# pkhungurn/talking-head-anime-4-demo

Hardware: NVIDIA H100
Metric: 512x512 RGBA frames/sec (higher is better)
Workload: dtype f16/tf32 operands (10-bit mantissa), f32 accumulate, f32 storage outside conv operands

## Files before the change

### include/tha4_b200.h

```cpp
#ifndef THA4_B200_H
#define THA4_B200_H

#include <stdint.h>

#ifdef __cplusplus
extern "C" {
#endif

typedef struct tha4_ctx tha4_ctx;

#define THA4_OK 0
#define THA4_ERR_INVALID (-1)
#define THA4_ERR_CUDA (-2)

enum tha4_net {
    THA4_NET_EYEBROW_DECOMPOSER = 0,
    THA4_NET_EYEBROW_MORPHING_COMBINER = 1,
    THA4_NET_FACE_MORPHER = 2,
    THA4_NET_BODY_MORPHER = 3,
    THA4_NET_UPSCALER = 4,
    THA4_NET_SIREN_FACE_MORPHER = 5,
    THA4_NET_SIREN_BODY_MORPHER = 6,
    THA4_NET_COUNT = 7
};
// ... 55 lines not shown
                                       int B, void* stream);
int tha4_siren_morpher_backward(tha4_ctx* ctx, const float* image, const float* pose, int pose_ld, int B,
                                const float* const* grad_outputs, const float* grid_change, const float* alpha,
                                const float* params, float* grads, float* d_image, float* d_pose, void* stream);
int tha4_siren_face_morpher_backward(tha4_ctx* ctx, const float* pose, int pose_ld, int B, const float* grad_output,
                                     const float* params, float* grads, float* d_pose, void* stream);
int tha4_adam_step(tha4_ctx* ctx, float* params, const float* grads, float* exp_avg, float* exp_avg_sq, int64_t n, float lr,
                   float beta1, float beta2, float eps, int step, float grad_scale, void* stream);

int tha4_images_differ(tha4_ctx* ctx, const float* a, const float* b, int64_t n, int* differ, void* stream);

int tha4_frame_to_srgb8(tha4_ctx* ctx, const float* frame, int B, int H, int W, int background, int round_mode, uint8_t* out, void* stream);
int tha4_rgba8_to_poser_image(tha4_ctx* ctx, const uint8_t* rgba, int H, int W, float* out, void* stream);

int tha4_grid_sample(tha4_ctx* ctx, const float* image, const float* grid_change, int N, int C, int H, int W,
                     float* out, int32_t* x0, int32_t* y0, float* tx, float* ty, void* stream);
int tha4_resize_bilinear(tha4_ctx* ctx, const float* in, int N, int C, int Hi, int Wi, int Ho, int Wo, float* out, void* stream);
int tha4_base_grid(int size, float* host_out);
int tha4_test_conv(tha4_ctx* ctx, int kind, const float* x, const float* w, const float* bias, const float* res,
                   int res_mode, int in_up, float* y, int N, int Cin, int H, int W, int Cout, int strict, int ksplit,
                   void* stream);
int tha4_test_conv_norm(tha4_ctx* ctx, int kind, const float* x, int N, int Cin, int H, int W, int norm_C, int groups,
                        const float* gamma, const float* beta, const float* film0, const float* film1, int act,
                        const float* w, const float* bias, const float* res, int res_mode, int Cout, int ksplit,
                        float* y, float* y_from_f16, void* stream);
int tha4_test_conv_norm_ex(tha4_ctx* ctx, int kind, const float* x, int N, int Cin, int H, int W, int norm_C, int groups,
                           const float* gamma, const float* beta, const float* film0, const float* film1, int act,
                           const float* w, const float* bias, const float* res, int res_mode, int Cout, int ksplit,
                           float* y, float* y_from_f16, double* y_stats, int reps, float* us_per_launch, void* stream);
int tha4_test_conv_skip_fold(tha4_ctx* ctx, const float* x, int N, int Cmid, int H, int W, int groups, const float* gamma,
                             const float* beta, const float* film0, const float* film1, int act, const float* w, const float* bias,
                             const float* x2, int Cin2, const float* w_skip, const float* b_skip, int Cout, int ksplit,
                             float* y, double* y_stats, int* folded, int reps, float* us_per_launch, void* stream);
int tha4_test_norm(tha4_ctx* ctx, const float* x, int N, int C, int H, int W, int groups, const float* gamma,
                   const float* beta, const float* film0, const float* film1, int act, int pool, int out_f16, float* y, void* stream);
int tha4_test_tail(tha4_ctx* ctx, int kind, const float* feature, int N, int C, int S, const float* gamma, const float* beta,
                   int groups, int act, const float* head_w, const float* head_b, const int* head_cout, int n_heads,
                   const float* image0, const float* image1, float* const* outputs, int strict, void* stream);
int tha4_test_conv_backward_data(tha4_ctx* ctx, int kind, const float* dy, const float* w, float* dx, int N, int Cin, int H, int W,
                                 int Cout, int strict, void* stream);
int tha4_test_norm_backward(tha4_ctx* ctx, const float* x, int N, int C, int H, int W, const float* gamma, const float* beta,
                            int act, const float* dy, float* dx, void* stream);
int tha4_test_tail_backward(tha4_ctx* ctx, int kind, const float* const* outputs, int N, int S, const float* image0,
                            const float* image1, const float* const* grad_outputs, float* d_head, float* d_image0,
                            float* d_image1, void* stream);
int tha4_test_upscaler_prologue_backward(tha4_ctx* ctx, const float* rest_image, const float* coarse_grid_change, int coarse_size,
                                         int N, const float* d_x0, float* d_rest_image, float* d_coarse_posed_image,
                                         float* d_coarse_grid_change, void* stream);
int tha4_test_group_norm_backward(tha4_ctx* ctx, const float* x, int N, int C, int H, int W, int groups, const float* gamma,
                                  const float* beta, const float* film0, const float* film1, int act, const float* dy, float* dx,
                                  float* d_film, void* stream);
int tha4_test_attention_backward(tha4_ctx* ctx, const float* qkv, const float* dout, int N, int C, int heads, float* dqkv, void* stream);
int tha4_test_group_norm_backward_ex(tha4_ctx* ctx, const void* x, int x_f16, int x_ld, int N, int C, int H, int W, int groups,
                                     const double* stats, int stats_rep, int stats_ld, const float* gamma, const float* beta,
                                     const float* film0, const float* film1, int film1_ld, int film1_off, int act, const float* dy,
                                     int dy_ld, int dy_pool, const float* res, int res_ld, int res_mode, const float* add, int add_ld,
                                     float* dx, int dx_ld, float* d_film, int d_film_ld, void* stream);
int tha4_test_norm_backward_ex(tha4_ctx* ctx, const void* x, int x_f16, int x_ld, int N, int C, int H, int W, const double* stats,
                               int stats_rep, int stats_ld, const float* gamma, const float* beta, int act, const float* dy, int dy_ld,
                               float* dx, int dx_ld, void* stream);
int tha4_test_conv_backward_data_ex(tha4_ctx* ctx, int kind, const float* w, const float* head_b, const int* head_cout, int n_heads,
                                    const float* dy, int dy_ld, const float* add, int add_ld, float* dx, int dx_ld, int N, int Cin,
                                    int H, int W, int Cout, int strict, int workspace, int* split_plan, void* stream);
int tha4_test_linear_backward(tha4_ctx* ctx, const float* dy, int dy_ld, int N, int R, const float* W, int K, const float* pre, int pre_ld,
                              float* dx, int dx_ld, void* stream);
int tha4_test_attention(tha4_ctx* ctx, const float* qkv, int N, int C, int heads, float* out, void* stream);
// ... 26 lines not shown
```

### tha4_b200/_lib.py

```python
import ctypes
import os
import weakref
from typing import Dict, List, Optional, Sequence

import torch
from torch import Tensor

_HERE = os.path.dirname(os.path.abspath(__file__))
LIB_PATH = os.path.join(_HERE, 'libtha4_b200.so')

NET_IDS = {
    'eyebrow_decomposer': 0, 'eyebrow_morphing_combiner': 1, 'face_morpher': 2, 'body_morpher': 3, 'upscaler': 4,
    'siren_face_morpher': 5, 'siren_body_morpher': 6,
}

EXPORTED_SYMBOLS = [
    'tha4_ctx_create', 'tha4_ctx_destroy', 'tha4_last_error', 'tha4_set_option', 'tha4_get_counter', 'tha4_load_net',
    'tha4_eyebrow_decomposer_forward', 'tha4_eyebrow_morphing_combiner_forward', 'tha4_face_morpher_forward',
    'tha4_morpher_forward', 'tha4_upscaler_forward', 'tha4_siren_face_morpher_forward', 'tha4_siren_morpher_forward',
    'tha4_teacher_forward', 'tha4_student_forward', 'tha4_student_forward_io',
    'tha4_bank_create', 'tha4_bank_destroy', 'tha4_bank_set_character', 'tha4_bank_forward', 'tha4_siren_morpher_param_count', 'tha4_siren_morpher_train_step',
    'tha4_siren_face_morpher_param_count', 'tha4_siren_face_morpher_train_step',
    'tha4_siren_morpher_backward', 'tha4_siren_face_morpher_backward',
    'tha4_adam_step', 'tha4_images_differ', 'tha4_frame_to_srgb8', 'tha4_rgba8_to_poser_image', 'tha4_grid_sample', 'tha4_resize_bilinear',
    'tha4_eyebrow_decomposer_backward', 'tha4_eyebrow_morphing_combiner_backward', 'tha4_face_morpher_backward',
    'tha4_morpher_backward', 'tha4_upscaler_backward',
    'tha4_test_conv_backward_data', 'tha4_test_norm_backward', 'tha4_test_tail_backward', 'tha4_test_upscaler_prologue_backward',
    'tha4_test_group_norm_backward', 'tha4_test_attention_backward',
    'tha4_test_group_norm_backward_ex', 'tha4_test_norm_backward_ex', 'tha4_test_conv_backward_data_ex', 'tha4_test_linear_backward',
    'tha4_base_grid', 'tha4_test_conv', 'tha4_test_conv_norm', 'tha4_test_conv_norm_ex', 'tha4_test_conv_skip_fold', 'tha4_test_norm', 'tha4_test_tail', 'tha4_test_attention', 'tha4_test_linear',
    'tha4_test_siren_level', 'tha4_test_sine', 'tha4_test_siren_plan_check',
    'tha4_test_dense_gemm', 'tha4_test_dense_wgrad', 'tha4_test_level_input', 'tha4_test_distill_sine', 'tha4_test_pose_grad',
    'tha4_test_distill_tail',
]

_lib = None


class Tha4Error(RuntimeError):
    pass


def load_library() -> ctypes.CDLL:
    global _lib
    if _lib is not None:
        return _lib
    if not os.path.exists(LIB_PATH):
        raise Tha4Error('tha4_b200: %s is missing -- build it with `python __graft_entry__.py` (nvcc, sm_100a). '
                        'There is no CPU / PyTorch fallback.' % LIB_PATH)
    lib = ctypes.CDLL(LIB_PATH)
    lib.tha4_last_error.restype = ctypes.c_char_p
    lib.tha4_last_error.argtypes = [ctypes.c_void_p]
    lib.tha4_get_counter.restype = ctypes.c_int64
    lib.tha4_get_counter.argtypes = [ctypes.c_void_p, ctypes.c_char_p]
    lib.tha4_set_option.argtypes = [ctypes.c_void_p, ctypes.c_char_p, ctypes.c_int64]
    lib.tha4_siren_morpher_param_count.restype = ctypes.c_int64
    lib.tha4_siren_face_morpher_param_count.restype = ctypes.c_int64
    lib.tha4_adam_step.argtypes = [ctypes.c_void_p, ctypes.c_void_p, ctypes.c_void_p, ctypes.c_void_p, ctypes.c_void_p, ctypes.c_int64,
                                   ctypes.c_float, ctypes.c_float, ctypes.c_float, ctypes.c_float, ctypes.c_int, ctypes.c_float,
                                   ctypes.c_void_p]
    lib.tha4_images_differ.argtypes = [ctypes.c_void_p, ctypes.c_void_p, ctypes.c_void_p, ctypes.c_int64,
                                       ctypes.POINTER(ctypes.c_int), ctypes.c_void_p]
    P, I, I64 = ctypes.c_void_p, ctypes.c_int, ctypes.c_int64
# ... 461 lines not shown
```

### tha4_b200/csrc/capi.cu

```cuda
#include "../../include/tha4_b200.h"
#include "nets.cuh"
#include "siren.cuh"
#include "profiler.cuh"
#include "distill.cuh"
#include <atomic>
#include <cstring>
#include <map>
#include <tuple>
#include <vector>

namespace tha4 {
std::atomic<long> g_kernel_launches{0};
bool g_use_pdl = true;
thread_local AllocSink* g_alloc_sink = nullptr;
void* tracked_malloc(size_t bytes) {
    void* p = nullptr;
    THA4_CUDA_CHECK(cudaMalloc(&p, std::max<size_t>(bytes, 16)));
    if (g_alloc_sink) g_alloc_sink->ptrs.push_back(p);
    return p;
}
}

using namespace tha4;

// ... 198 lines not shown

int tha4_ctx_destroy(tha4_ctx* ctx) {
    if (!ctx) return THA4_ERR_INVALID;
    cudaSetDevice(ctx->device);
    cudaDeviceSynchronize();
    if (ctx->flag) cudaFree(ctx->flag);
    if (ctx->loss_acc) cudaFree(ctx->loss_acc);
    if (ctx->pose_stage) cudaFree(ctx->pose_stage);
    if (ctx->capture_stream) cudaStreamDestroy(ctx->capture_stream);
    if (ctx->side) { cudaStreamDestroy(ctx->side); cudaEventDestroy(ctx->ev_fork); cudaEventDestroy(ctx->ev_join); }
    if (ctx->stats_base) cudaFree(ctx->stats_base);
    ctx->drop_graphs();
    delete ctx;
    return THA4_OK;
}

const char* tha4_last_error(const tha4_ctx* ctx) { return ctx ? ctx->err.c_str() : g_create_err.c_str(); }

int tha4_set_option(tha4_ctx* ctx, const char* name, int64_t value) {
    return guarded(ctx, [&] {
        cudaDeviceSynchronize();
        ctx->drop_graphs();
        if (!strcmp(name, "strict")) { ctx->strict = value ? 1 : 0; }
        else if (!strcmp(name, "cuda_graphs")) ctx->use_graphs = value ? 1 : 0;
        else if (!strcmp(name, "side_stream")) ctx->side_streams = value ? 1 : 0;
        else if (!strcmp(name, "tcgen05")) conv_enable_tc(value != 0);
        else if (!strcmp(name, "cluster_splitk")) conv_tc_enable_cluster(value != 0);
        else if (!strcmp(name, "halo_conv")) conv_halo_enable(value != 0);
        else if (!strcmp(name, "tma_store")) conv_halo_enable_tma_store(value != 0);
        else if (!strcmp(name, "halo_m256")) { THA4_REQUIRE(value >= -1 && value <= 1, "halo_m256: -1, 0 or 1"); conv_halo_set_m256((int)value); }
        else if (!strcmp(name, "halo_ctas")) { THA4_REQUIRE(value == -1 || value == 1 || value == 2, "halo_ctas: -1, 1 or 2"); conv_halo_set_ctas((int)value); }
        else if (!strcmp(name, "halo_cs")) { THA4_REQUIRE(value == -1 || value == 1 || value == 2, "halo_cs: -1, 1 or 2"); conv_halo_set_cs((int)value); }
        else if (!strcmp(name, "skip_fold")) unet_set_skip_fold(value != 0);
        else if (!strcmp(name, "siren_tc")) siren_tc_enable(value != 0);
        else if (!strcmp(name, "tc_stride2")) conv_tc_enable_stride2(value != 0);
        else if (!strcmp(name, "small_bn")) conv_tc_enable_small_bn(value != 0);
        else if (!strcmp(name, "attn_split16")) attention_enable_split16(value != 0);
        else if (!strcmp(name, "tail_persist")) tail_tc_enable_persist(value != 0);
        else if (!strcmp(name, "attn_mma")) attention_enable_mma(value != 0);
        else if (!strcmp(name, "half_operands")) ctx->half_operands = value ? 1 : 0;
        else if (!strcmp(name, "pdl")) g_use_pdl = value != 0;
        else if (!strcmp(name, "profile")) { prof_enable(value != 0); if (value == 2) prof_reset(); }
        else if (!strcmp(name, "microbatch")) { THA4_REQUIRE(value >= 1 && value <= 1024, "microbatch range"); ctx->microbatch = (int)value; }
        else throw std::runtime_error(std::string("tha4: unknown option ") + name);
    });
}

int64_t tha4_get_counter(const tha4_ctx* ctx, const char* name) {
    if (!strcmp(name, "kernel_launches")) return g_kernel_launches.load();
    {
        static const char* cats[] = {"conv", "norm", "tail", "attn", "glue", "siren"};
        static const char* whats[] = {"us", "launches", "flops", "bytes"};
        if (!strncmp(name, "prof_", 5))
            for (int w = 0; w < 4; ++w)
                for (int c = 0; c < 6; ++c)
                    if (std::string(name) == std::string("prof_") + whats[w] + "_" + cats[c]) {
                        try { return (int64_t)prof_read(c, w); } catch (...) { return -1; }
                    }
    }
    if (ctx && !strcmp(name, "graph_replays")) return (int64_t)ctx->graph_replays;
    if (ctx && !strcmp(name, "graph_captures")) return (int64_t)ctx->graph_captures;
    if (ctx && !strcmp(name, "graph_failures")) return (int64_t)ctx->graph_failures;
    if (ctx && !strcmp(name, "workspace_bytes")) return (int64_t)(ctx->persist.bytes() + ctx->scratch.bytes());
    return -1;
}

// ... 687 lines not shown
        const bool fold = unet_skip_fold() && conv_halo_supported(fw, fa);
        View sk = mk(N, H, W, Cout);
        ConvArgs sa; sa.in = x16; sa.out = sk;
        a.res = sk; a.res_mode = RES_SAME;
        const size_t wsf = std::max(conv_workspace_floats(sw, sa), conv_workspace_floats(cw, a));
        float* ws = wsf ? ctx->scratch.alloc(wsf) : nullptr;
        for (ConvArgs* c : {&sa, &a}) { c->ws = ws; c->ws_floats = wsf; }
        auto run = [&] {
            if (fold) { conv_forward(fw, fa, s); return; }
            if (y_stats) THA4_CUDA_CHECK(cudaMemsetAsync(yo.stats, 0, (size_t)N * Cout * 2 * sizeof(double), s));
            conv_forward(sw, sa, s);
            conv_forward(cw, a, s);
        };
        run();
        if (y_stats) THA4_CUDA_CHECK(cudaMemcpyAsync(y_stats, yo.stats, (size_t)N * Cout * 2 * sizeof(double), cudaMemcpyDeviceToDevice, s));
        if (folded) *folded = fold ? 1 : 0;
        if (reps > 0) {
            cudaEvent_t e0, e1;
            THA4_CUDA_CHECK(cudaEventCreate(&e0)); THA4_CUDA_CHECK(cudaEventCreate(&e1));
            THA4_CUDA_CHECK(cudaEventRecord(e0, s));
            for (int i = 0; i < reps; ++i) run();
            THA4_CUDA_CHECK(cudaEventRecord(e1, s));
            THA4_CUDA_CHECK(cudaEventSynchronize(e1));
            float ms = 0.0f;
            THA4_CUDA_CHECK(cudaEventElapsedTime(&ms, e0, e1));
            cudaEventDestroy(e0); cudaEventDestroy(e1);
            if (us_per_launch) *us_per_launch = 1000.0f * ms / reps;
        }
        nhwc_to_nchw(yo, y, s);
        THA4_CUDA_CHECK(cudaStreamSynchronize(s));
    });
}

int tha4_test_norm(tha4_ctx* ctx, const float* x, int N, int C, int H, int W, int groups, const float* gamma,
                   const float* beta, const float* film0, const float* film1, int act, int pool, int out_f16, float* y, void* stream) {
    return guarded(ctx, [&] {
        cudaStream_t s = (cudaStream_t)stream;
        begin_pass(ctx, s);
        Runtime rt = make_rt(ctx, stream);
        Pool* P = &ctx->persist;
        View xin; xin.N = N; xin.H = H; xin.W = W; xin.C = C; xin.ld = C; xin.p = P->alloc((size_t)N * H * W * C);
        xin.stats_rep = 2; xin.stats_rep_stride = (long)N * C * 2;
        xin.stats = rt.alloc_stats((size_t)2 * N * C * 2); xin.stats_ld = C;
        nchw_to_nhwc(make_img(x, N, C, H, W), xin, s);
        norm_stats(xin, s);
        View yo = xin; yo.stats = nullptr;
        if (pool) { yo.H = H / 2; yo.W = W / 2; }
        yo.p = P->alloc((size_t)N * yo.H * yo.W * C);
        if (out_f16) {
            View y16 = yo; y16.f16 = 1; y16.p = P->alloc(((size_t)N * yo.H * yo.W * C + 1) / 2);
            norm_apply_fused(xin, groups, gamma, beta, film0, film1, 2 * C, act == ACT_SILU ? ACT_SILU_FAST : act, pool, nullptr, y16, s, 1);
            convert_f32(y16, yo, s);
        } else {
            norm_apply_fused(xin, groups, gamma, beta, film0, film1, 2 * C, act, pool, nullptr, yo, s, 0);
        }
        nhwc_to_nchw(yo, y, s);
    });
}

int tha4_test_tail(tha4_ctx* ctx, int kind, const float* feature, int N, int C, int S, const float* gamma, const float* beta,
                   int groups, int act, const float* head_w, const float* head_b, const int* head_cout, int n_heads,
                   const float* image0, const float* image1, float* const* outputs, int strict, void* stream) {
    return guarded(ctx, [&] {
        cudaStream_t s = (cudaStream_t)stream;
        begin_pass(ctx, s);
        Runtime rt = make_rt(ctx, stream);
// ... 405 lines not shown
```

### tha4_b200/csrc/conv.cuh

```cuda
#pragma once
#include "common.cuh"

namespace tha4 {

constexpr int CONV_MAX_TAPS = 16;
constexpr int CONV_MAX_PHASES = 4;

enum ResMode { RES_NONE = 0, RES_SAME = 1, RES_UP2 = 2, RES_DOWN2 = 3 };

struct ConvWeights {
    float* w = nullptr;
    mutable __half* w16 = nullptr;
    mutable float w16_scale = 1.0f;
    float* bias = nullptr;
    int cin = 0, cout = 0, cin_pad = 0, cout_pad = 0;
    int ntaps = 0, nphase = 1;
    bool dynamic = false;
    bool tf32_rounded = false;
    int stride = 1;
    int out_mul = 1;
    signed char dy[CONV_MAX_PHASES][CONV_MAX_TAPS];
    signed char dx[CONV_MAX_PHASES][CONV_MAX_TAPS];
    signed char ph_oy[CONV_MAX_PHASES], ph_ox[CONV_MAX_PHASES];
    int cin2 = 0, cin2_pad = 0;
// ... 30 lines not shown
    View res;
    int res_mode = RES_NONE;
    int strict = 0;
    int ksplit = 0;
    float* ws = nullptr;
    size_t ws_floats = 0;
};

size_t conv_workspace_floats(const ConvWeights& cw, const ConvArgs& a);

void conv_forward(const ConvWeights& cw, const ConvArgs& a, cudaStream_t s);
void conv_mma_forward(const ConvWeights& cw, const ConvArgs& a, cudaStream_t s);
bool conv_tc_supported(const ConvWeights& cw, const ConvArgs& a);
void conv_tc_forward(const ConvWeights& cw, const ConvArgs& a, cudaStream_t s);
bool conv_fuses_stats(const ConvWeights& cw, const ConvArgs& a);
bool conv_tc_fuses_stats(const ConvWeights& cw, const ConvArgs& a);
int conv_tc_split_plan(const ConvWeights& cw, const ConvArgs& a);
bool conv_halo_supported(const ConvWeights& cw, const ConvArgs& a);
void conv_halo_forward(const ConvWeights& cw, const ConvArgs& a, cudaStream_t s);
void conv_halo_enable(bool on);
void conv_halo_enable_tma_store(bool on);
void conv_halo_set_ctas(int mode);
void conv_halo_set_cs(int mode);
void conv_halo_set_m256(int mode);
void conv_halo_debug_dump();
void conv_enable_tc(bool on);
bool conv_tc_enabled();
void conv_make_half(const ConvWeights& cw, cudaStream_t s);
void conv_make_fold(ConvWeights& fold, const ConvWeights& conv3, const ConvWeights& conv1x1, cudaStream_t s);
void conv_tc_enable_cluster(bool on);
void conv_tc_enable_small_bn(bool on);
void conv_tc_enable_stride2(bool on);

}
```

### tha4_b200/csrc/nets.cu

```cuda
#include "nets.cuh"
#include <algorithm>
#include <cmath>
#include <cstdlib>

namespace tha4 {

Pool::~Pool() { for (void* p : all_) cudaFree(p); }

float* Pool::alloc(size_t nfloats) {
    size_t bytes = ((nfloats * sizeof(float) + 255) / 256) * 256;
    if (bytes == 0) bytes = 256;
    Bucket& bk = buckets_[bytes];
    if (bk.next < bk.blocks.size()) return reinterpret_cast<float*>(bk.blocks[bk.next++]);
    void* p = nullptr;
    THA4_CUDA_CHECK(cudaMalloc(&p, bytes));
    bk.blocks.push_back(p);
    bk.next = bk.blocks.size();
    all_.push_back(p);
    total_ += bytes;
    return reinterpret_cast<float*>(p);
}

void Pool::reset() { for (auto& kv : buckets_) kv.second.next = 0; }

// ... 670 lines not shown
                rt.stream = rt.side;
                try { run_conv_tc(rt, w.skip, x.h, nullptr, sk); } catch (...) { rt.stream = main_stream; throw; }
                rt.stream = main_stream;
                THA4_CUDA_CHECK(cudaEventRecord(rt.ev_join, rt.side));
            } else {
                run_conv_tc(rt, w.skip, x.h, nullptr, sk);
            }
        }
        View xpool;
        if (mode == 2) {
            View t0 = make_view16(rt.scratch, B, x.f.H / 2, x.f.W / 2, w.cin);
            xpool = make_view(rt.scratch, B, x.f.H / 2, x.f.W / 2, w.cin);
            run_norm(rt, x.f, w.norm0, 32, nullptr, nullptr, 0, act, 1, nullptr, t0, nullptr, &xpool);
            run_conv_tc(rt, w.conv0, t0, nullptr, h0);
        } else {
            const ConvNormIn n0 = norm_in(x.f, w.norm0, 32, act);
            run_conv_tc(rt, w.conv0, x.h, &n0, h0);
        }
        const ConvNormIn n1 = norm_in(h0.f, w.norm1, 32, act, w.film0, film1 + w.film1_off, film1_total);
        if (fold) {
            run_conv_tc(rt, w.fold, h0.h, &n1, out, nullptr, RES_NONE, &x.h);
        } else if (w.has_skip) {
            THA4_REQUIRE(mode == 0, "res_block: skip conv only on same-resolution blocks");
            if (rt.side) THA4_CUDA_CHECK(cudaStreamWaitEvent(rt.stream, rt.ev_join, 0));
            run_conv_tc(rt, w.conv1, h0.h, &n1, out, &sk.f, RES_SAME);
        } else {
            if (mode == 2) run_conv_tc(rt, w.conv1, h0.h, &n1, out, &xpool, RES_SAME);
            else run_conv_tc(rt, w.conv1, h0.h, &n1, out, &x.f, mode == 0 ? RES_SAME : RES_UP2);
        }
    }

    void attn_block(const AttnW& w, const Tens& x, const Tens& out) {
        rt.scratch->reset();
        Tens qkv = make_act(tape ? rt.persist : rt.scratch, rt, x.f.N, x.f.H, x.f.W, 3 * x.f.C, true, false, false);
        const ConvNormIn n = norm_in(x.f, w.norm, 32, ACT_NONE);
        run_conv_tc(rt, w.qkv, x.h, &n, qkv);
        if (tape) tape->attn[&w] = {op_view(x), qkv.f};
        View a = make_view(rt.scratch, x.f.N, x.f.H, x.f.W, x.f.C);
        attention_forward(qkv.f, 8, a, rt.stream, true);
        run_conv_tc(rt, w.proj, a, nullptr, out, &x.f, RES_SAME);
    }
};

}

void UNetNet::forward_fused(Runtime& rt, const ImgView& image, const float* coarse_posed, const float* coarse_grid, int coarse_size,
                            const float* pose, int pose_ld, float* const* outputs, UNetTape* tape) {
    const int B = image.N;
    cudaStream_t s = rt.stream;
    Pool* P = rt.persist;
    rt.scratch->reset();

    float* c1 = P->alloc((size_t)B * 256);
    float* c2 = P->alloc((size_t)B * 256);
    float* film1 = P->alloc((size_t)B * film1_total_);
    cudaStream_t ls = s;
    if (rt.side) {
        THA4_CUDA_CHECK(cudaEventRecord(rt.ev_fork, s));
        THA4_CUDA_CHECK(cudaStreamWaitEvent(rt.side, rt.ev_fork, 0));
        ls = rt.side;
    }
    linear_forward(pose, pose_ld, B, 6, cond_w0_, cond_b0_, 256, 0, c1, 256, ls);
    linear_forward(c1, 256, B, 256, cond_w2_, cond_b2_, 256, 1, c2, 256, ls);
    linear_forward(c2, 256, B, 256, film1_w_, film1_b_, film1_total_, 1, film1, film1_total_, ls);
    if (rt.side) THA4_CUDA_CHECK(cudaEventRecord(rt.ev_join, rt.side));
    if (tape) { tape->c1 = c1; tape->c2 = c2; tape->film1 = film1; }
    UNetFused F{rt, film1, film1_total_, tape};

// ... 99 lines not shown
```

Before: 178.7.

## Fuse attention block into one clustered kernel with DSMEM K/V exchange

Replaces the three-launch attention block (norm plus qkv 1x1 conv, attention, proj conv plus residual) with a single kernel. It runs a 16-CTA cluster per image, one CTA per head and half of the tokens, and uses distributed shared memory to exchange K/V halves and per-head outputs before the projection. It also writes output stats and the f16 copy in the epilogue. The goal is to avoid the round trips of qkv and attention output through global memory and to save launch overhead, at the cost of a fixed 16x16x256 shape and a large cluster that may not place well.

Result: faster. 183.7 (median of 6 runs) (+2.8%).

```diff
diff --git a/include/tha4_b200.h b/include/tha4_b200.h
--- a/include/tha4_b200.h
+++ b/include/tha4_b200.h
@@ -111,6 +111,10 @@
                              const float* beta, const float* film0, const float* film1, int act, const float* w, const float* bias,
                              const float* x2, int Cin2, const float* w_skip, const float* b_skip, int Cout, int ksplit,
                              float* y, double* y_stats, int* folded, int reps, float* us_per_launch, void* stream);
+int tha4_test_attn_block(tha4_ctx* ctx, const float* x, int N, int in_reps, const float* gamma, const float* beta,
+                         const float* w_qkv, const float* b_qkv, const float* w_proj, const float* b_proj, int out_mode, int out_ld,
+                         int out_reps, float* y, float* y16, double* y_stats, float* qkv, int* fused, int reps, float* us_per_launch,
+                         void* stream);
 int tha4_test_norm(tha4_ctx* ctx, const float* x, int N, int C, int H, int W, int groups, const float* gamma,
                    const float* beta, const float* film0, const float* film1, int act, int pool, int out_f16, float* y, void* stream);
 int tha4_test_tail(tha4_ctx* ctx, int kind, const float* feature, int N, int C, int S, const float* gamma, const float* beta,
diff --git a/tha4_b200/_lib.py b/tha4_b200/_lib.py
--- a/tha4_b200/_lib.py
+++ b/tha4_b200/_lib.py
@@ -28,7 +28,7 @@
     'tha4_test_conv_backward_data', 'tha4_test_norm_backward', 'tha4_test_tail_backward', 'tha4_test_upscaler_prologue_backward',
     'tha4_test_group_norm_backward', 'tha4_test_attention_backward',
     'tha4_test_group_norm_backward_ex', 'tha4_test_norm_backward_ex', 'tha4_test_conv_backward_data_ex', 'tha4_test_linear_backward',
-    'tha4_base_grid', 'tha4_test_conv', 'tha4_test_conv_norm', 'tha4_test_conv_norm_ex', 'tha4_test_conv_skip_fold', 'tha4_test_norm', 'tha4_test_tail', 'tha4_test_attention', 'tha4_test_linear',
+    'tha4_base_grid', 'tha4_test_conv', 'tha4_test_conv_norm', 'tha4_test_conv_norm_ex', 'tha4_test_conv_skip_fold', 'tha4_test_attn_block', 'tha4_test_norm', 'tha4_test_tail', 'tha4_test_attention', 'tha4_test_linear',
     'tha4_test_siren_level', 'tha4_test_sine', 'tha4_test_siren_plan_check',
     'tha4_test_dense_gemm', 'tha4_test_dense_wgrad', 'tha4_test_level_input', 'tha4_test_distill_sine', 'tha4_test_pose_grad',
     'tha4_test_distill_tail',
diff --git a/tha4_b200/csrc/attention_block.cu b/tha4_b200/csrc/attention_block.cu
--- /dev/null
+++ b/tha4_b200/csrc/attention_block.cu
@@ -0,0 +1,363 @@
+#include "conv.cuh"
+#include "ops.cuh"
+#include "profiler.cuh"
+#include "conv_tc_device.cuh"
+
+namespace tha4 {
+namespace {
+
+constexpr int AB_L = 256, AB_C = 256, AB_D = 32, AB_HEADS = 8;
+constexpr int AB_CS = 2 * AB_HEADS;
+constexpr int AB_T = AB_L / 2;
+constexpr int AB_THREADS = 256;
+constexpr int XP = AB_C + 8;
+constexpr int KH_P = AB_D + 8, VT_P = AB_L + 8;
+constexpr int SM_X = 0;
+constexpr int SM_Q = SM_X + AB_T * XP * 2;
+constexpr int SM_K = SM_Q + AB_T * KH_P * 2;
+constexpr int SM_VT = SM_K + AB_L * KH_P * 2;
+constexpr int SM_WQ = SM_VT + AB_D * VT_P * 2;
+constexpr int SM_WP = SM_WQ + 3 * AB_D * XP * 2;
+constexpr int SM_HA = SM_WP + AB_D * XP * 2;
+constexpr int SM_CHS = SM_HA + 2 * AB_C * 2;
+constexpr int SM_RED = SM_CHS + AB_C * 16;
+constexpr int SM_BYTES = SM_RED + 8 * AB_D * 8;
+static_assert(SM_BYTES <= 227 * 1024, "shared memory budget");
+static_assert(3 * AB_D * XP >= AB_T * KH_P, "O_h staging fits in the qkv weight rows");
+
+struct AbParams {
+    tcdev::TcParams xf;
+    const __half* x; int x_ld;
+    const __half* wq; int wq_ld; const float* bq; float sq;
+    const __half* wp; int wp_ld; const float* bp; float sp;
+    const float* res; int res_ld;
+    float* out; int out_ld;
+    __half* out16; int out16_ld;
+    double* stats; int stats_ld, stats_rep; long stats_rep_stride;
+    float* qkv; int qkv_ld;
+    int pre_w;
+};
+
+__device__ __forceinline__ uint32_t pack_h2(float a, float b) {
+    const __half2 h = __floats2half2_rn(a, b);
+    return *reinterpret_cast<const uint32_t*>(&h);
+}
+__device__ __forceinline__ void mma_16816(float (&c)[4], const uint32_t (&a)[4], uint32_t b0, uint32_t b1) {
+    asm volatile("mma.sync.aligned.m16n8k16.row.col.f32.f16.f16.f32 {%0, %1, %2, %3}, {%4, %5, %6, %7}, {%8, %9}, {%0, %1, %2, %3};\n"
+                 : "+f"(c[0]), "+f"(c[1]), "+f"(c[2]), "+f"(c[3]) : "r"(a[0]), "r"(a[1]), "r"(a[2]), "r"(a[3]), "r"(b0), "r"(b1));
+}
+__device__ __forceinline__ void cp_async16(uint32_t dst, const void* src) {
+    asm volatile("cp.async.cg.shared.global [%0], [%1], 16;\n" :: "r"(dst), "l"(src) : "memory");
+}
+__device__ __forceinline__ void cluster_sync() {
+    asm volatile("barrier.cluster.arrive.release.aligned;\n" ::: "memory");
+    asm volatile("barrier.cluster.wait.acquire.aligned;\n" ::: "memory");
+}
+__device__ __forceinline__ uint32_t peer_addr(uint32_t local, int rank) {
+    uint32_t r;
+    asm volatile("mapa.shared::cluster.u32 %0, %1, %2;\n" : "=r"(r) : "r"(local), "r"(rank));
+    return r;
+}
+__device__ __forceinline__ float tf32_trunc(float v) { return __uint_as_float(__float_as_uint(v) & 0xffffe000u); }
+
+__global__ void __launch_bounds__(AB_THREADS, 1) attn_block_kernel(const __grid_constant__ AbParams p) {
+    extern __shared__ __align__(16) uint8_t sm[];
+    const int tid = threadIdx.x, warp = tid >> 5, lane = tid & 31, g = lane >> 2, t = lane & 3;
+    const int rank = blockIdx.z % AB_CS, n = blockIdx.z / AB_CS;
+    const int h = rank % AB_HEADS, half = rank / AB_HEADS, partner = rank ^ AB_HEADS;
+    const int t0 = half * AB_T;
+    const uint32_t s_base = tc::smem_u32(sm);
+    asm volatile("barrier.cluster.arrive.relaxed.aligned;\n" ::: "memory");
+
+    auto load_w = [&] {
+        for (int j = tid; j < 4 * AB_D * (AB_C / 8); j += AB_THREADS) {
+            const int r = j >> 5, c8 = (j & 31) * 8;
+            if (r < 3 * AB_D) {
+                const __half* src = p.wq + (long)((r >> 5) * AB_C + h * AB_D + (r & 31)) * p.wq_ld + c8;
+                cp_async16(s_base + SM_WQ + (r * XP + c8) * 2, src);
+            } else {
+                const int rp = r - 3 * AB_D;
+                cp_async16(s_base + SM_WP + (rp * XP + c8) * 2, p.wp + (long)(h * AB_D + rp) * p.wp_ld + c8);
+            }
+        }
+        asm volatile("cp.async.commit_group;\n" ::: "memory");
+    };
+    if (p.pre_w) load_w();
+    pdl_trigger();
+    pdl_wait();
+    if (!p.pre_w) load_w();
+
+    {
+        const __half* xs = p.x + ((long)n * AB_L + t0) * p.x_ld;
+        for (int j = tid; j < AB_T * (AB_C / 8); j += AB_THREADS) {
+            const int r = j >> 5, c8 = (j & 31) * 8;
+            cp_async16(s_base + SM_X + (r * XP + c8) * 2, xs + (long)r * p.x_ld + c8);
+        }
+        asm volatile("cp.async.commit_group;\n" ::: "memory");
+    }
+    __half* hA = reinterpret_cast<__half*>(sm + SM_HA);
+    __half* hB = hA + AB_C;
+    tcdev::xf_build_coef<AB_THREADS, 1>(p.xf, n, tid, hA, hB, reinterpret_cast<double2*>(sm + SM_CHS), 0, AB_C);
+    asm volatile("cp.async.wait_all;\n" ::: "memory");
+    __syncthreads();
+    {
+        uint8_t* row = sm + SM_X + (tid >> 1) * XP * 2;
+        const int j0 = (tid & 1) * 16;
+        tcdev::xf_chunks<8>(row, 0, j0, 0, p.xf, hA, hB, false);
+        tcdev::xf_chunks<8>(row, 0, j0 + 8, 0, p.xf, hA, hB, false);
+    }
+    __syncthreads();
+
+    const uint32_t* xw = reinterpret_cast<const uint32_t*>(sm + SM_X);
+    const int m0 = 16 * warp;
+    {
+        float acc[12][4];
+#pragma unroll
+        for (int nj = 0; nj < 12; ++nj) acc[nj][0] = acc[nj][1] = acc[nj][2] = acc[nj][3] = 0.0f;
+        const uint32_t* ww = reinterpret_cast<const uint32_t*>(sm + SM_WQ);
+#pragma unroll 2
+        for (int ks = 0; ks < AB_C / 16; ++ks) {
+            uint32_t a[4];
+            const int lo = (m0 + g) * (XP / 2) + 8 * ks + t, hi = lo + 8 * (XP / 2);
+            a[0] = xw[lo]; a[1] = xw[hi]; a[2] = xw[lo + 4]; a[3] = xw[hi + 4];
+#pragma unroll
+            for (int nj = 0; nj < 12; ++nj) {
+                const int br = (8 * nj + g) * (XP / 2) + 8 * ks + t;
+                mma_16816(acc[nj], a, ww[br], ww[br + 4]);
+            }
+        }
+        const float scale = 1.0f / sqrtf(sqrtf((float)AB_D));
+        uint32_t* qw = reinterpret_cast<uint32_t*>(sm + SM_Q);
+        asm volatile("barrier.cluster.wait.aligned;\n" ::: "memory");
+#pragma unroll
+        for (int nj = 0; nj < 12; ++nj) {
+            const int part = nj >> 2, d = 8 * (nj & 3) + 2 * t;
+            const int gch = part * AB_C + h * AB_D + d;
+            const float b0 = __ldg(p.bq + gch), b1 = __ldg(p.bq + gch + 1);
+#pragma unroll
+            for (int e = 0; e < 2; ++e) {
+                const int rl = m0 + g + 8 * e, r = t0 + rl;
+                const float v0 = acc[nj][2 * e] * p.sq + b0, v1 = acc[nj][2 * e + 1] * p.sq + b1;
+                if (p.qkv) *reinterpret_cast<float2*>(p.qkv + ((long)n * AB_L + r) * p.qkv_ld + gch) = make_float2(v0, v1);
+                if (part == 0) {
+                    qw[(rl * KH_P + d) >> 1] = pack_h2(v0 * scale, v1 * scale);
+                } else if (part == 1) {
+                    const uint32_t kv = pack_h2(v0 * scale, v1 * scale);
+                    const uint32_t a = s_base + SM_K + (r * KH_P + d) * 2;
+                    asm volatile("st.shared.b32 [%0], %1;\n" :: "r"(a), "r"(kv) : "memory");
+                    asm volatile("st.shared::cluster.b32 [%0], %1;\n" :: "r"(peer_addr(a, partner)), "r"(kv) : "memory");
+                } else {
+                    const __half2 vh = __floats2half2_rn(v0, v1);
+                    const unsigned short u0 = __half_as_ushort(__low2half(vh)), u1 = __half_as_ushort(__high2half(vh));
+                    const uint32_t a0 = s_base + SM_VT + (d * VT_P + r) * 2, a1 = a0 + VT_P * 2;
+                    asm volatile("st.shared.b16 [%0], %1;\n" :: "r"(a0), "h"(u0) : "memory");
+                    asm volatile("st.shared.b16 [%0], %1;\n" :: "r"(a1), "h"(u1) : "memory");
+                    asm volatile("st.shared::cluster.b16 [%0], %1;\n" :: "r"(peer_addr(a0, partner)), "h"(u0) : "memory");
+                    asm volatile("st.shared::cluster.b16 [%0], %1;\n" :: "r"(peer_addr(a1, partner)), "h"(u1) : "memory");
+                }
+            }
+        }
+    }
+    cluster_sync();
+
+    {
+        const uint32_t* qw = reinterpret_cast<const uint32_t*>(sm + SM_Q);
+        const uint32_t* kw = reinterpret_cast<const uint32_t*>(sm + SM_K);
+        const uint32_t* vw = reinterpret_cast<const uint32_t*>(sm + SM_VT);
+        uint32_t* os = reinterpret_cast<uint32_t*>(sm + SM_WQ);
+        const int q0 = m0;
+        uint32_t qa[2][4];
+#pragma unroll
+        for (int ks = 0; ks < 2; ++ks) {
+            const int lo = ((q0 + g) * KH_P) / 2 + 8 * ks + t, hi = ((q0 + g + 8) * KH_P) / 2 + 8 * ks + t;
+            qa[ks][0] = qw[lo]; qa[ks][1] = qw[hi]; qa[ks][2] = qw[lo + 4]; qa[ks][3] = qw[hi + 4];
+        }
+        float sc[AB_L / 8][4];
+#pragma unroll
+        for (int j = 0; j < AB_L / 8; ++j) {
+            sc[j][0] = sc[j][1] = sc[j][2] = sc[j][3] = 0.0f;
+            const int krow = ((8 * j + g) * KH_P) >> 1;
+#pragma unroll
+            for (int ks = 0; ks < 2; ++ks)
+                mma_16816(sc[j], qa[ks], kw[krow + 8 * ks + t], kw[krow + 8 * ks + t + 4]);
+        }
+        float mx0 = -INFINITY, mx1 = -INFINITY;
+#pragma unroll
+        for (int j = 0; j < AB_L / 8; ++j) { mx0 = fmaxf(mx0, fmaxf(sc[j][0], sc[j][1])); mx1 = fmaxf(mx1, fmaxf(sc[j][2], sc[j][3])); }
+        mx0 = fmaxf(mx0, __shfl_xor_sync(0xffffffffu, mx0, 1)); mx0 = fmaxf(mx0, __shfl_xor_sync(0xffffffffu, mx0, 2));
+        mx1 = fmaxf(mx1, __shfl_xor_sync(0xffffffffu, mx1, 1)); mx1 = fmaxf(mx1, __shfl_xor_sync(0xffffffffu, mx1, 2));
+        float l0 = 0.0f, l1 = 0.0f;
+        constexpr float LOG2E = 1.4426950408889634f;
+        const float mb0 = mx0 * LOG2E, mb1 = mx1 * LOG2E;
+#pragma unroll
+        for (int j = 0; j < AB_L / 8; ++j) {
+            sc[j][0] = exp2f(fmaf(sc[j][0], LOG2E, -mb0)); sc[j][1] = exp2f(fmaf(sc[j][1], LOG2E, -mb0));
+            sc[j][2] = exp2f(fmaf(sc[j][2], LOG2E, -mb1)); sc[j][3] = exp2f(fmaf(sc[j][3], LOG2E, -mb1));
+            l0 += sc[j][0] + sc[j][1]; l1 += sc[j][2] + sc[j][3];
+        }
+        l0 += __shfl_xor_sync(0xffffffffu, l0, 1); l0 += __shfl_xor_sync(0xffffffffu, l0, 2);
+        l1 += __shfl_xor_sync(0xffffffffu, l1, 1); l1 += __shfl_xor_sync(0xffffffffu, l1, 2);
+        float oc[AB_D / 8][4];
+#pragma unroll
+        for (int nd = 0; nd < AB_D / 8; ++nd) oc[nd][0] = oc[nd][1] = oc[nd][2] = oc[nd][3] = 0.0f;
+#pragma unroll
+        for (int kk = 0; kk < AB_L / 16; ++kk) {
+            uint32_t pa[4];
+            pa[0] = pack_h2(sc[2 * kk][0], sc[2 * kk][1]); pa[1] = pack_h2(sc[2 * kk][2], sc[2 * kk][3]);
+            pa[2] = pack_h2(sc[2 * kk + 1][0], sc[2 * kk + 1][1]); pa[3] = pack_h2(sc[2 * kk + 1][2], sc[2 * kk + 1][3]);
+#pragma unroll
+            for (int nd = 0; nd < AB_D / 8; ++nd) {
+                const int vrow = ((8 * nd + g) * VT_P + 16 * kk) >> 1;
+                mma_16816(oc[nd], pa, vw[vrow + t], vw[vrow + t + 4]);
+            }
+        }
+        const float i0 = 1.0f / l0, i1 = 1.0f / l1;
+#pragma unroll
+        for (int nd = 0; nd < AB_D / 8; ++nd) {
+            os[((q0 + g) * KH_P + 8 * nd + 2 * t) >> 1] = pack_h2(tf32_trunc(oc[nd][0] * i0), tf32_trunc(oc[nd][1] * i0));
+            os[((q0 + g + 8) * KH_P + 8 * nd + 2 * t) >> 1] = pack_h2(tf32_trunc(oc[nd][2] * i1), tf32_trunc(oc[nd][3] * i1));
+        }
+    }
+    __syncthreads();
+
+    for (int j = tid; j < AB_T * (AB_D / 8); j += AB_THREADS) {
+        const int r = j >> 2, c4 = j & 3;
+        const uint4 v = *reinterpret_cast<const uint4*>(sm + SM_WQ + (r * KH_P + 8 * c4) * 2);
+        const uint32_t local = s_base + SM_X + (r * XP + h * AB_D + 8 * c4) * 2;
+#pragma unroll
+        for (int rk = 0; rk < AB_HEADS; ++rk)
+            asm volatile("st.shared::cluster.v4.b32 [%0], {%1, %2, %3, %4};\n"
+                         :: "r"(peer_addr(local, rk + AB_HEADS * half)), "r"(v.x), "r"(v.y), "r"(v.z), "r"(v.w) : "memory");
+    }
+    cluster_sync();
+
+    float acc[4][4];
+#pragma unroll
+    for (int nj = 0; nj < 4; ++nj) acc[nj][0] = acc[nj][1] = acc[nj][2] = acc[nj][3] = 0.0f;
+    {
+        const uint32_t* ww = reinterpret_cast<const uint32_t*>(sm + SM_WP);
+#pragma unroll 4
+        for (int ks = 0; ks < AB_C / 16; ++ks) {
+            uint32_t a[4];
+            const int lo = (m0 + g) * (XP / 2) + 8 * ks + t, hi = lo + 8 * (XP / 2);
+            a[0] = xw[lo]; a[1] = xw[hi]; a[2] = xw[lo + 4]; a[3] = xw[hi + 4];
+#pragma unroll
+            for (int nj = 0; nj < 4; ++nj) {
+                const int br = (8 * nj + g) * (XP / 2) + 8 * ks + t;
+                mma_16816(acc[nj], a, ww[br], ww[br + 4]);
+            }
+        }
+    }
+    float su[4][2], sq[4][2];
+#pragma unroll
+    for (int nj = 0; nj < 4; ++nj) {
+        const int ch = h * AB_D + 8 * nj + 2 * t;
+        const float b0 = __ldg(p.bp + ch), b1 = __ldg(p.bp + ch + 1);
+        su[nj][0] = su[nj][1] = sq[nj][0] = sq[nj][1] = 0.0f;
+#pragma unroll
+        for (int e = 0; e < 2; ++e) {
+            const long pix = (long)n * AB_L + t0 + m0 + g + 8 * e;
+            const float2 rr = *reinterpret_cast<const float2*>(p.res + pix * p.res_ld + ch);
+            float v0 = acc[nj][2 * e] * p.sp, v1 = acc[nj][2 * e + 1] * p.sp;
+            v0 += b0; v1 += b1;
+            v0 += rr.x; v1 += rr.y;
+            if (p.out) *reinterpret_cast<float2*>(p.out + pix * p.out_ld + ch) = make_float2(v0, v1);
+            if (p.out16) *reinterpret_cast<__half2*>(p.out16 + pix * p.out16_ld + ch) = __floats2half2_rn(v0, v1);
+            su[nj][0] += v0; su[nj][1] += v1; sq[nj][0] += v0 * v0; sq[nj][1] += v1 * v1;
+        }
+    }
+    if (p.stats) {
+        float2* red = reinterpret_cast<float2*>(sm + SM_RED);
+#pragma unroll
+        for (int nj = 0; nj < 4; ++nj)
+#pragma unroll
+            for (int c = 0; c < 2; ++c) {
+                float a = su[nj][c], b = sq[nj][c];
+#pragma unroll
+                for (int off = 4; off < 32; off <<= 1) { a += __shfl_xor_sync(0xffffffffu, a, off); b += __shfl_xor_sync(0xffffffffu, b, off); }
+                if (g == 0) red[warp * AB_D + 8 * nj + 2 * t + c] = make_float2(a, b);
+            }
+        __syncthreads();
+        if (tid < AB_D) {
+            double a = 0.0, b = 0.0;
+#pragma unroll
+            for (int w = 0; w < AB_THREADS / 32; ++w) { const float2 v = red[w * AB_D + tid]; a += (double)v.x; b += (double)v.y; }
+            double* d = p.stats + (long)(blockIdx.z % p.stats_rep) * p.stats_rep_stride + ((long)n * p.stats_ld + h * AB_D + tid) * 2;
+            atomicAdd(d, a); atomicAdd(d + 1, b);
+        }
+    }
+}
+
+bool g_attn_fuse = true;
+
+int max_clusters() {
+    static int n[THA4_MAX_DEVICES];
+    static bool known[THA4_MAX_DEVICES];
+    const int d = current_device();
+    if (!known[d]) {
+        THA4_CUDA_CHECK(cudaFuncSetAttribute(attn_block_kernel, cudaFuncAttributeMaxDynamicSharedMemorySize, SM_BYTES));
+        THA4_CUDA_CHECK(cudaFuncSetAttribute(attn_block_kernel, cudaFuncAttributeNonPortableClusterSizeAllowed, 1));
+        cudaLaunchConfig_t cfg{};
+        cfg.gridDim = dim3(1, 1, AB_CS); cfg.blockDim = dim3(AB_THREADS); cfg.dynamicSmemBytes = SM_BYTES;
+        cudaLaunchAttribute attr;
+        attr.id = cudaLaunchAttributeClusterDimension;
+        attr.val.clusterDim.x = 1; attr.val.clusterDim.y = 1; attr.val.clusterDim.z = AB_CS;
+        cfg.attrs = &attr; cfg.numAttrs = 1;
+        int c = 0;
+        if (cudaOccupancyMaxActiveClusters(&c, attn_block_kernel, &cfg) != cudaSuccess) { (void)cudaGetLastError(); c = 0; }
+        n[d] = c; known[d] = true;
+    }
+    return n[d];
+}
+
+}
+
+void attn_block_enable_fuse(bool on) { g_attn_fuse = on; }
+
+bool attn_block_fused_for(int N) { return g_attn_fuse && N <= max_clusters(); }
+
+void attn_block_forward(const ConvWeights& qkv, const ConvWeights& proj, const View& x16, const ConvNormIn& nin, const View& res,
+                        const View& out, const View& out16, const View* qkv_out, cudaStream_t s) {
+    THA4_REQUIRE(x16.f16 && x16.H * x16.W == AB_L && x16.C == AB_C, "attn_block: the input is an f16 view of 256 tokens x 256 channels");
+    THA4_REQUIRE(qkv.ntaps == 1 && qkv.nphase == 1 && qkv.cin == AB_C && qkv.cout == 3 * AB_C && proj.ntaps == 1 && proj.nphase == 1 &&
+                 proj.cin == AB_C && proj.cout == AB_C && AB_C / AB_HEADS == AB_D, "attn_block: 1x1 convs 256 -> 768 and 256 -> 256, 8 heads of 32");
+    THA4_REQUIRE(qkv.w16 && proj.w16 && qkv.bias && proj.bias, "attn_block: the f16 weight copies and the biases");
+    THA4_REQUIRE(qkv.cin_pad % 8 == 0 && proj.cin_pad % 8 == 0 && (((uintptr_t)qkv.w16) & 15) == 0 && (((uintptr_t)proj.w16) & 15) == 0,
+                 "attn_block: weight alignment");
+    THA4_REQUIRE(x16.ld % 8 == 0 && (((uintptr_t)x16.p) & 15) == 0, "attn_block: input alignment (16-byte rows)");
+    THA4_REQUIRE(nin.on && nin.C == AB_C && nin.groups > 0 && AB_C % nin.groups == 0 && nin.stats && nin.gamma && nin.beta &&
+                 !nin.film0 && !nin.film1, "attn_block: a pending GroupNorm of the input");
+    THA4_REQUIRE(res.p && !res.f16 && res.N == x16.N && res.H * res.W == AB_L && res.C == AB_C && res.ld % 2 == 0 && (((uintptr_t)res.p) & 7) == 0,
+                 "attn_block: fp32 residual geometry / alignment");
+    THA4_REQUIRE(out.p || out16.p, "attn_block: no output");
+    THA4_REQUIRE(out.N == x16.N && out.H * out.W == AB_L && out.C == AB_C, "attn_block: output geometry");
+    if (out.p) THA4_REQUIRE(!out.f16 && out.ld % 2 == 0 && (((uintptr_t)out.p) & 7) == 0, "attn_block: fp32 output alignment");
+    if (out16.p)
+        THA4_REQUIRE(out16.f16 && out16.N == out.N && out16.H * out16.W == AB_L && out16.C == AB_C && out16.ld % 2 == 0 &&
+                     (((uintptr_t)out16.p) & 3) == 0, "attn_block: f16 output geometry / alignment");
+    if (qkv_out) THA4_REQUIRE(!qkv_out->f16 && qkv_out->N == x16.N && qkv_out->H * qkv_out->W == AB_L && qkv_out->C == 3 * AB_C &&
+                              qkv_out->ld % 2 == 0 && (((uintptr_t)qkv_out->p) & 7) == 0, "attn_block: qkv output geometry / alignment");
+    AbParams p{};
+    p.xf.in_stats = nin.stats; p.xf.in_stats_ld = nin.stats_ld; p.xf.in_stats_rep = std::max(1, nin.stats_rep);
+    p.xf.in_stats_rep_stride = nin.stats_rep_stride;
+    p.xf.xf_C = AB_C; p.xf.xf_groups = nin.groups; p.xf.xf_act = nin.act;
+    THA4_REQUIRE(nin.act == ACT_NONE, "attn_block: GroupNorm without activation");
+    p.xf.xf_inv_cnt = 1.0 / ((double)AB_L * (AB_C / nin.groups));
+    p.xf.xf_gamma = nin.gamma; p.xf.xf_beta = nin.beta;
+    p.x = x16.hp(); p.x_ld = x16.ld;
+    p.wq = qkv.w16; p.wq_ld = qkv.cin_pad; p.bq = qkv.bias; p.sq = 1.0f / qkv.w16_scale;
+    p.wp = proj.w16; p.wp_ld = proj.cin_pad; p.bp = proj.bias; p.sp = 1.0f / proj.w16_scale;
+    p.res = res.p; p.res_ld = res.ld;
+    p.out = out.p; p.out_ld = out.ld;
+    p.out16 = out16.p ? out16.hp() : nullptr; p.out16_ld = out16.ld;
+    p.stats = out.stats; p.stats_ld = out.stats_ld; p.stats_rep = std::max(1, out.stats_rep); p.stats_rep_stride = out.stats_rep_stride;
+    p.qkv = qkv_out ? qkv_out->p : nullptr; p.qkv_ld = qkv_out ? qkv_out->ld : 0;
+    p.pre_w = (qkv.dynamic || proj.dynamic) ? 0 : 1;
+    ProfScope prof(PROF_ATTN, s);
+    prof_add_work(PROF_ATTN, (double)x16.N * (2.0 * AB_L * AB_C * 4 * AB_C + 4.0 * AB_L * AB_L * AB_C), 0.0);
+    THA4_REQUIRE(max_clusters() > 0, "attn_block: the device cannot place a 16-CTA cluster of this kernel");
+    launch_pdl(attn_block_kernel, dim3(1, 1, AB_CS * x16.N), dim3(AB_THREADS), SM_BYTES, s, AB_CS, p);
+    THA4_LAUNCH_CHECK();
+}
+
+}
diff --git a/tha4_b200/csrc/capi.cu b/tha4_b200/csrc/capi.cu
--- a/tha4_b200/csrc/capi.cu
+++ b/tha4_b200/csrc/capi.cu
@@ -254,6 +254,7 @@
         else if (!strcmp(name, "halo_ctas")) { THA4_REQUIRE(value == -1 || value == 1 || value == 2, "halo_ctas: -1, 1 or 2"); conv_halo_set_ctas((int)value); }
         else if (!strcmp(name, "halo_cs")) { THA4_REQUIRE(value == -1 || value == 1 || value == 2, "halo_cs: -1, 1 or 2"); conv_halo_set_cs((int)value); }
         else if (!strcmp(name, "skip_fold")) unet_set_skip_fold(value != 0);
+        else if (!strcmp(name, "attn_fuse")) attn_block_enable_fuse(value != 0);
         else if (!strcmp(name, "siren_tc")) siren_tc_enable(value != 0);
         else if (!strcmp(name, "tc_stride2")) conv_tc_enable_stride2(value != 0);
         else if (!strcmp(name, "small_bn")) conv_tc_enable_small_bn(value != 0);
@@ -1007,6 +1008,92 @@
     });
 }
 
+int tha4_test_attn_block(tha4_ctx* ctx, const float* x, int N, int in_reps, const float* gamma, const float* beta,
+                         const float* w_qkv, const float* b_qkv, const float* w_proj, const float* b_proj, int out_mode, int out_ld,
+                         int out_reps, float* y, float* y16, double* y_stats, float* qkv, int* fused, int reps, float* us_per_launch,
+                         void* stream) {
+    return guarded(ctx, [&] {
+        cudaStream_t s = (cudaStream_t)stream;
+        begin_pass(ctx, s);
+        Runtime rt = make_rt(ctx, stream);
+        Pool* P = &ctx->persist;
+        constexpr int C = 256, HW = 16;
+        THA4_REQUIRE(N >= 1 && in_reps >= 1 && out_reps >= 1 && out_ld >= C && out_ld % 8 == 0 && (out_mode & 3) != 0,
+                     "test_attn_block: arguments");
+        AllocSink sink;
+        ConvWeights wq, wp;
+        {
+            SinkScope own(&sink);
+            conv_set_pack_rounding(true);
+            for (int k = 0; k < 2; ++k) {
+                ConvWeights& c = k ? wp : wq;
+                conv_describe(c, CONV_1x1, C, k ? C : 3 * C);
+                c.tf32_rounded = true;
+                c.w = reinterpret_cast<float*>(tracked_malloc(conv_packed_floats(c) * sizeof(float)));
+                THA4_CUDA_CHECK(cudaMemsetAsync(c.w, 0, conv_packed_floats(c) * sizeof(float), s));
+                conv_pack(c, CONV_1x1, k ? w_proj : w_qkv, C, 0, s);
+                conv_make_half(c, s);
+            }
+        }
+        wq.bias = const_cast<float*>(b_qkv); wp.bias = const_cast<float*>(b_proj);
+        View xin; xin.N = N; xin.H = HW; xin.W = HW; xin.C = C; xin.ld = C; xin.p = P->alloc((size_t)N * HW * HW * C);
+        xin.stats_rep = in_reps; xin.stats_rep_stride = (long)N * C * 2; xin.stats_ld = C;
+        xin.stats = rt.alloc_stats((size_t)in_reps * N * C * 2);
+        THA4_CUDA_CHECK(cudaMemsetAsync(xin.stats, 0, (size_t)in_reps * N * C * 2 * sizeof(double), s));
+        THA4_CUDA_CHECK(cudaMemcpyAsync(xin.p, x, (size_t)N * HW * HW * C * sizeof(float), cudaMemcpyDeviceToDevice, s));
+        norm_stats(xin, s);
+        View x16 = xin; x16.f16 = 1; x16.stats = nullptr; x16.p = P->alloc((size_t)N * HW * HW * C / 2);
+        convert_f16(xin, x16, s);
+        const size_t on = (size_t)N * HW * HW * out_ld;
+        View of; of.N = N; of.H = HW; of.W = HW; of.C = out_ld; of.ld = out_ld; of.p = P->alloc(on);
+        View oh = of; oh.f16 = 1; oh.p = P->alloc(on / 2);
+        THA4_CUDA_CHECK(cudaMemsetAsync(of.p, 0xff, on * sizeof(float), s));
+        THA4_CUDA_CHECK(cudaMemsetAsync(oh.p, 0xff, on * sizeof(__half), s));
+        const size_t stn = (size_t)out_reps * N * out_ld * 2;
+        of.stats = rt.alloc_stats(stn); of.stats_ld = out_ld; of.stats_rep = out_reps; of.stats_rep_stride = (long)N * out_ld * 2;
+        View o32 = of.slice(out_ld - C, C), o16 = oh.slice(out_ld - C, C);
+        if (!(out_mode & 1)) o32.p = nullptr;
+        if (!(out_mode & 2)) o16.p = nullptr;
+        ConvNormIn nin;
+        nin.on = true; nin.C = C; nin.groups = 32; nin.act = ACT_NONE; nin.gamma = gamma; nin.beta = beta;
+        nin.stats = xin.stats; nin.stats_ld = C; nin.stats_rep = in_reps; nin.stats_rep_stride = xin.stats_rep_stride;
+        View qv; qv.N = N; qv.H = HW; qv.W = HW; qv.C = 3 * C; qv.ld = 3 * C; qv.p = P->alloc((size_t)N * HW * HW * 3 * C);
+        View av = xin; av.stats = nullptr; av.p = P->alloc((size_t)N * HW * HW * C);
+        const bool fuse = attn_block_fused_for(N);
+        ConvArgs a; a.in = x16; a.out = qv; a.nin = nin;
+        ConvArgs b; b.in = av; b.out = o32; b.out16 = o16; b.res = xin; b.res_mode = RES_SAME;
+        const size_t wsf = std::max(conv_workspace_floats(wq, a), conv_workspace_floats(wp, b));
+        float* ws = wsf ? ctx->scratch.alloc(wsf) : nullptr;
+        for (ConvArgs* c : {&a, &b}) { c->ws = ws; c->ws_floats = wsf; }
+        auto run = [&] {
+            THA4_CUDA_CHECK(cudaMemsetAsync(of.stats, 0, stn * sizeof(double), s));
+            if (fuse) { attn_block_forward(wq, wp, x16, nin, xin, o32, o16, qkv ? &qv : nullptr, s); return; }
+            conv_forward(wq, a, s);
+            attention_forward(qv, 8, av, s, true);
+            conv_forward(wp, b, s);
+        };
+        run();
+        if (fused) *fused = fuse ? 1 : 0;
+        if (reps > 0) {
+            cudaEvent_t e0, e1;
+            THA4_CUDA_CHECK(cudaEventCreate(&e0)); THA4_CUDA_CHECK(cudaEventCreate(&e1));
+            THA4_CUDA_CHECK(cudaEventRecord(e0, s));
+            for (int i = 0; i < reps; ++i) run();
+            THA4_CUDA_CHECK(cudaEventRecord(e1, s));
+            THA4_CUDA_CHECK(cudaEventSynchronize(e1));
+            float ms = 0.0f;
+            THA4_CUDA_CHECK(cudaEventElapsedTime(&ms, e0, e1));
+            cudaEventDestroy(e0); cudaEventDestroy(e1);
+            if (us_per_launch) *us_per_launch = 1000.0f * ms / reps;
+        }
+        if (y) THA4_CUDA_CHECK(cudaMemcpyAsync(y, of.p, on * sizeof(float), cudaMemcpyDeviceToDevice, s));
+        if (y16) { View t = of; t.stats = nullptr; t.p = y16; convert_f32(oh, t, s); }
+        if (y_stats) THA4_CUDA_CHECK(cudaMemcpyAsync(y_stats, of.stats, stn * sizeof(double), cudaMemcpyDeviceToDevice, s));
+        if (qkv) THA4_CUDA_CHECK(cudaMemcpyAsync(qkv, qv.p, (size_t)N * HW * HW * 3 * C * sizeof(float), cudaMemcpyDeviceToDevice, s));
+        THA4_CUDA_CHECK(cudaStreamSynchronize(s));
+    });
+}
+
 int tha4_test_norm(tha4_ctx* ctx, const float* x, int N, int C, int H, int W, int groups, const float* gamma,
                    const float* beta, const float* film0, const float* film1, int act, int pool, int out_f16, float* y, void* stream) {
     return guarded(ctx, [&] {
diff --git a/tha4_b200/csrc/conv.cuh b/tha4_b200/csrc/conv.cuh
--- a/tha4_b200/csrc/conv.cuh
+++ b/tha4_b200/csrc/conv.cuh
@@ -86,4 +86,9 @@
 void conv_tc_enable_small_bn(bool on);
 void conv_tc_enable_stride2(bool on);
 
+void attn_block_forward(const ConvWeights& qkv, const ConvWeights& proj, const View& x16, const ConvNormIn& nin, const View& res,
+                        const View& out, const View& out16, const View* qkv_out, cudaStream_t s);
+void attn_block_enable_fuse(bool on);
+bool attn_block_fused_for(int N);
+
 }
diff --git a/tha4_b200/csrc/nets.cu b/tha4_b200/csrc/nets.cu
--- a/tha4_b200/csrc/nets.cu
+++ b/tha4_b200/csrc/nets.cu
@@ -726,8 +726,15 @@
 
     void attn_block(const AttnW& w, const Tens& x, const Tens& out) {
         rt.scratch->reset();
+        const ConvNormIn n = norm_in(x.f, w.norm, 32, ACT_NONE);
+        if (attn_block_fused_for(x.f.N)) {
+            View qkv;
+            if (tape) qkv = make_view(rt.persist, x.f.N, x.f.H, x.f.W, 3 * x.f.C);
+            attn_block_forward(w.qkv, w.proj, x.h, n, x.f, out.f, out.h, tape ? &qkv : nullptr, rt.stream);
+            if (tape) tape->attn[&w] = {op_view(x), qkv};
+            return;
+        }
         Tens qkv = make_act(tape ? rt.persist : rt.scratch, rt, x.f.N, x.f.H, x.f.W, 3 * x.f.C, true, false, false);
-        const ConvNormIn n = norm_in(x.f, w.norm, 32, ACT_NONE);
         run_conv_tc(rt, w.qkv, x.h, &n, qkv);
         if (tape) tape->attn[&w] = {op_view(x), qkv.f};
         View a = make_view(rt.scratch, x.f.N, x.f.H, x.f.W, x.f.C);
```
